# Tencent-RoboticsX/lifelike-agility-and-play

Hardware: NVIDIA H100
Metric: env-steps/sec PMC mocap-tracking (higher is better)
Workload: dtype f32

## Files before the change

lifelike_agility_and_play_b200/csrc/llq_cuda.cu:

```cuda
#include "../../include/llq.h"
#include "../../include/llq_model_layout.h"
#include "llq_kernels.cuh"
#include "llq_step16.cuh"

#include <cmath>
#include <cstdio>
#include <cstdlib>
#include <cstring>
#include <new>
#include <string>
#include <vector>

namespace {

thread_local std::string g_err;
int fail(int code, const std::string& msg) { g_err = msg; return code; }
#define CK(call)                                                                                         \
  do {                                                                                                   \
    cudaError_t e_ = (call);                                                                             \
    if (e_ != cudaSuccess) return fail(LLQ_ECUDA, std::string(#call) + ": " + cudaGetErrorString(e_));   \
  } while (0)

constexpr int kPadFrames = 128;

// ... 48 lines not shown
  P.sim_dt = c.sim_dt; P.frame_dt = h->frame_dt; P.margin = h->margin;
  P.max_steps = c.max_steps; P.cmd_freq_lo = c.cmd_freq_lo; P.cmd_freq_hi = c.cmd_freq_hi; P.push_start_count = c.push_start_count;
  P.push_interval = c.push_interval_steps; P.push_duration = c.push_duration_steps; P.push_enabled = c.push_enabled;
  P.mu_ground = (float)c.ground_friction; P.fr_lo = (float)c.friction_lo; P.fr_hi = (float)c.friction_hi;
  P.ph_lo = (float)c.push_h_lo; P.ph_hi = (float)c.push_h_hi; P.pv_lo = (float)c.push_v_lo; P.pv_hi = (float)c.push_v_hi;
  P.ts_lo = (float)c.target_spd_lo; P.ts_hi = (float)c.target_spd_hi;
  P.knee = c.knee_contacts; P.mu_wheel = (float)(c.ground_friction * c.link_friction); P.aux_r = (float)c.auxiliary_radius;
  P.element_id = c.element_id; P.ww_lo = (float)c.wall_width_lo; P.ww_hi = (float)c.wall_width_hi; P.wg_lo = (float)c.wall_gap_lo;
  P.wg_hi = (float)c.wall_gap_hi; P.hg_lo = (float)c.hole_gap_lo; P.hg_hi = (float)c.hole_gap_hi;
  if (!h->has_obstacles) { P.has_ob = 0; P.ob_hx = P.ob_hy = P.ob_hz = 0.f; }
}

template <typename T> int dalloc(T** p, size_t n) {
  CK(cudaMalloc((void**)p, n * sizeof(T)));
  CK(cudaMemset(*p, 0, n * sizeof(T)));
  return LLQ_OK;
}

int ensure_scratch(llq_handle h, size_t bytes) {
  if (bytes > h->h_scratch_bytes) {
    if (h->h_scratch) cudaFreeHost(h->h_scratch);
    if (h->d_scratch) cudaFree(h->d_scratch);
    h->h_scratch = nullptr; h->d_scratch = nullptr; h->h_scratch_bytes = 0;
    CK(cudaMallocHost(&h->h_scratch, bytes));
    CK(cudaMalloc(&h->d_scratch, bytes));
    h->h_scratch_bytes = h->d_scratch_bytes = bytes;
  }
  return LLQ_OK;
}

llq::MocapDev mocap_dev(llq_handle h) { return llq::MocapDev{h->d_frames, h->d_clip_off, h->n_clips, h->d_ob_table, h->d_ob_off}; }

template <int ENV>
void launch_reset_t(llq_handle h, const llq::EnvArrays& E, const llq::ResetParams& RP, float* obs2, long long ld, cudaStream_t s) {
  constexpr int BLOCK = llq::kResetBlock;
  int threads = 4 * h->cfg.n_envs;
  int grid = (threads + BLOCK - 1) / BLOCK;
  size_t smem = sizeof(double) * (size_t)(h->n_clips > 0 ? h->n_clips : 1);
  llq::pmc_reset_kernel<ENV><<<grid, BLOCK, smem, s>>>(E, mocap_dev(h), h->P, h->d_model, RP, obs2, ld);
}
template <int ENV>
int launch_step16(llq_handle h, const llq::EnvArrays& E, const float* a, float* obs2, long long ld, cudaStream_t s) {
  constexpr int EPB = LLQ16_BLOCK / 16;
  const int grid = (h->cfg.n_envs + EPB - 1) / EPB;
  const size_t smem = sizeof(float) * (EPB * llq::kEnvFloats + (LLQ16_BLOCK / 32) * llq::kATabWarp);
  const unsigned bit = 1u << (16 + ENV);
  if (!(h->smem_attr_set & bit)) {
    CK(cudaFuncSetAttribute(llq::llq_step16_kernel<ENV>, cudaFuncAttributeMaxDynamicSharedMemorySize, (int)smem));
    h->smem_attr_set |= bit;
  }
  llq::llq_step16_kernel<ENV><<<grid, LLQ16_BLOCK, smem, s>>>(E, mocap_dev(h), h->P, h->d_model, h->d_sph, a, obs2, ld, h->d_winner[h->parity],
                                                   (unsigned long long)h->cfg.seed, (long long)h->cfg.global_env_offset, h->record);
  return LLQ_OK;
}
int launch_step(llq_handle h, const llq::EnvArrays& E, const float* a, float* obs2, long long ld, cudaStream_t s) {
  const bool epmc = h->cfg.env_kind == LLQ_ENV_EPMC;
  h->counters[4]++;
  if (epmc && h->cfg.element_id != 0) return launch_step16<3>(h, E, a, obs2, ld, s);
  if (h->cfg.env_kind == LLQ_ENV_SEPMC) return launch_step16<2>(h, E, a, obs2, ld, s);
  return epmc ? launch_step16<1>(h, E, a, obs2, ld, s) : launch_step16<0>(h, E, a, obs2, ld, s);
}
void launch_reset(llq_handle h, const llq::EnvArrays& E, const llq::ResetParams& RP, float* obs2, long long ld, cudaStream_t s) {
  if (h->cfg.env_kind == LLQ_ENV_EPMC && h->cfg.element_id != 0) launch_reset_t<3>(h, E, RP, obs2, ld, s);
  else if (h->cfg.env_kind == LLQ_ENV_EPMC) launch_reset_t<1>(h, E, RP, obs2, ld, s);
  else if (h->cfg.env_kind == LLQ_ENV_SEPMC) launch_reset_t<2>(h, E, RP, obs2, ld, s);
  else launch_reset_t<0>(h, E, RP, obs2, ld, s);
  h->counters[4]++;
}

llq::ResetParams reset_params(llq_handle h, int mode, bool update_table) {
  llq::ResetParams RP{};
  RP.mode = mode; RP.mask = nullptr; RP.clip_in = nullptr; RP.time_in = nullptr;
  RP.seed = h->cfg.seed; RP.gid0 = h->cfg.global_env_offset;
  RP.winner_cur = h->d_winner[h->parity]; RP.winner_next = h->d_winner[h->parity ^ 1];
  RP.avg_old = h->d_avg[h->parity]; RP.avg_new = update_table ? h->d_avg[h->parity ^ 1] : h->d_avg[h->parity];
  RP.prob = h->d_prob; RP.max_steps = h->d_max_steps; RP.factor = h->cfg.prioritized_sample_factor;
  RP.update_table = update_table ? 1 : 0;
  return RP;
}

int check_ready(llq_handle h, bool need_reset) {
  if (!h) return fail(LLQ_EINVAL, "null handle");
  if (!h->has_model) return fail(LLQ_ESTATE, "llq_load_model has not been called");
  if (h->cfg.env_kind == LLQ_ENV_PMC && !h->has_mocap) return fail(LLQ_ESTATE, "llq_load_mocap has not been called");
  if (h->cfg.env_kind != LLQ_ENV_PMC && !h->has_init_state) return fail(LLQ_ESTATE, "llq_set_init_state has not been called");
  if (need_reset && !h->was_reset) return fail(LLQ_ESTATE, "llq_reset has not been called");
  return set_device(h);
}

void copy_item(llq::DampItem& d, const double* s) {
  d.m = (float)s[0];
  for (int i = 0; i < 3; i++) d.c[i] = (float)s[1 + i];
  for (int i = 0; i < 6; i++) d.Ic[i] = (float)s[4 + i];
}

int get_soa_f(llq_handle h, const float* d_src, int width, float* dst) {
  const int n = h->cfg.n_envs;
  int rc = ensure_scratch(h, sizeof(float) * (size_t)width * n);
  if (rc) return rc;
  CK(cudaMemcpyAsync(h->h_scratch, d_src, sizeof(float) * (size_t)width * n, cudaMemcpyDeviceToHost, h->stream));
// ... 287 lines not shown
  const size_t total = (size_t)offsets[n_clips];
  CK(cudaMalloc((void**)&h->d_ob_table, sizeof(double) * 4 * (total ? total : 1)));
  if (total) CK(cudaMemcpy(h->d_ob_table, table, sizeof(double) * 4 * total, cudaMemcpyHostToDevice));
  CK(cudaMalloc((void**)&h->d_ob_off, sizeof(int) * (n_clips + 1)));
  CK(cudaMemcpy(h->d_ob_off, offsets, sizeof(int) * (n_clips + 1), cudaMemcpyHostToDevice));
  h->has_obstacles = true;
  h->P.has_ob = 1; h->P.ob_hx = (float)hx; h->P.ob_hy = (float)hy; h->P.ob_hz = (float)hz;
  return LLQ_OK;
}

static int do_reset(llq_handle h, const uint8_t* mask, const int32_t* clip, const double* time, float* obs) {
  const size_t n = (size_t)h->cfg.n_envs;
  llq::ResetParams RP = reset_params(h, clip ? 2 : 1, false);
  if (mask) {
    std::memcpy(h->h_done, mask, n);
    CK(cudaMemcpyAsync(h->d_mask, h->h_done, n, cudaMemcpyHostToDevice, h->stream));
    RP.mask = h->d_mask;
  }
  if (clip) {
    for (size_t i = 0; i < n; i++) {
      if (mask && !mask[i]) continue;
      if (clip[i] < 0 || clip[i] >= h->n_clips) return fail(LLQ_EINVAL, "clip id out of range");
      int nf = h->clip_off[clip[i] + 1] - h->clip_off[clip[i]];
      if (!(time[i] >= 0) || time[i] >= h->frame_dt * (nf - h->margin - 1)) return fail(LLQ_EINVAL, "reset time outside clip");
    }
    int rc = ensure_scratch(h, n * (sizeof(int) + sizeof(double)));
    if (rc) return rc;
    double* ht = (double*)h->h_scratch; int* hc = (int*)(ht + n);
    std::memcpy(ht, time, n * sizeof(double)); std::memcpy(hc, clip, n * sizeof(int));
    CK(cudaMemcpyAsync(h->d_time_in, ht, n * sizeof(double), cudaMemcpyHostToDevice, h->stream));
    CK(cudaMemcpyAsync(h->d_clip_in, hc, n * sizeof(int), cudaMemcpyHostToDevice, h->stream));
    RP.clip_in = h->d_clip_in; RP.time_in = h->d_time_in;
  }
  launch_reset(h, h->E, RP, nullptr, h->obs_dim, h->stream);
  CK(cudaGetLastError());
  if (obs) CK(cudaMemcpyAsync(h->h_obs, h->E.obs, sizeof(float) * h->obs_dim * n, cudaMemcpyDeviceToHost, h->stream));
  CK(cudaStreamSynchronize(h->stream));
  if (obs) std::memcpy(obs, h->h_obs, sizeof(float) * h->obs_dim * n);
  h->was_reset = true;
  return LLQ_OK;
}

int llq_reset(llq_handle h, const uint8_t* mask, float* obs) {
  int rc = check_ready(h, false);
  if (rc) return rc;
  return do_reset(h, mask, nullptr, nullptr, obs);
}

int llq_reset_to(llq_handle h, const uint8_t* mask, const int32_t* clip, const double* time, float* obs) {
  int rc = check_ready(h, false);
  if (rc) return rc;
  if (h->cfg.env_kind != LLQ_ENV_PMC) return fail(LLQ_EUNSUPPORTED, "llq_reset_to is a PMC (mocap) entry point");
  if (!clip || !time) return fail(LLQ_EINVAL, "null clip/time");
  return do_reset(h, mask, clip, time, obs);
}

int llq_step_ex(llq_handle h, const float* actions, float* obs, int64_t obs_ld, float* reward, uint8_t* done, int io_mode,
                void* stream) {
  int rc = check_ready(h, true);
  if (rc) return rc;
  if (!actions) return fail(LLQ_EINVAL, "null actions");
  const size_t od = (size_t)h->obs_dim;
  if (obs && obs_ld < (int64_t)od) return fail(LLQ_EINVAL, "obs_ld smaller than the observation width");
  if (h->record && io_mode == LLQ_IO_DEVICE && obs && obs_ld < (int64_t)od + 14)
    return fail(LLQ_EINVAL, "record mode needs obs_ld >= observation width + 14 (action 12 | reward | done)");
  const size_t n = (size_t)h->cfg.n_envs;
  llq::EnvArrays E = h->E;
  const float* d_act;
  float* obs2 = nullptr;
  cudaStream_t s = h->stream;
  if (io_mode == LLQ_IO_DEVICE) {
    if (stream) s = (cudaStream_t)stream;
    d_act = actions;
    if (reward) E.reward = reward;
    if (done) E.done = done;
    obs2 = obs;
  } else if (io_mode == LLQ_IO_HOST) {
    std::memcpy(h->h_actions, actions, sizeof(float) * LLQ_ACTION_DIM * n);
    CK(cudaMemcpyAsync(h->d_actions, h->h_actions, sizeof(float) * LLQ_ACTION_DIM * n, cudaMemcpyHostToDevice, s));
    d_act = h->d_actions;
  } else if (io_mode == LLQ_IO_PINNED) {
    CK(cudaMemcpyAsync(h->d_actions, actions, sizeof(float) * LLQ_ACTION_DIM * n, cudaMemcpyHostToDevice, s));
    d_act = h->d_actions;
  } else {
    return fail(LLQ_EINVAL, "bad io_mode");
  }
  if (h->profile) CK(cudaEventRecord(h->ev[0], s));
  rc = launch_step(h, E, d_act, obs2, (long long)obs_ld, s);
  if (rc) return rc;
  if (h->profile) CK(cudaEventRecord(h->ev[1], s));
  llq::ResetParams RP = reset_params(h, h->cfg.auto_reset ? 0 : 3, true);
  launch_reset(h, E, RP, obs2, (long long)obs_ld, s);
  if (h->profile) { CK(cudaEventRecord(h->ev[2], s)); h->ev_valid = true; }
  h->parity ^= 1;
  CK(cudaGetLastError());
  h->counters[0] += (int64_t)n;
  if (io_mode == LLQ_IO_HOST) {
    if (obs) CK(cudaMemcpyAsync(h->h_obs, h->E.obs, sizeof(float) * od * n, cudaMemcpyDeviceToHost, s));
    if (reward) CK(cudaMemcpyAsync(h->h_reward, h->E.reward, sizeof(float) * n, cudaMemcpyDeviceToHost, s));
    if (done) CK(cudaMemcpyAsync(h->h_done, h->E.done, n, cudaMemcpyDeviceToHost, s));
    CK(cudaStreamSynchronize(s));
    if (obs) {
      if ((size_t)obs_ld == od) std::memcpy(obs, h->h_obs, sizeof(float) * od * n);
      else for (size_t i = 0; i < n; i++) std::memcpy(obs + i * obs_ld, h->h_obs + i * od, sizeof(float) * od);
    }
    if (reward) std::memcpy(reward, h->h_reward, sizeof(float) * n);
    if (done) std::memcpy(done, h->h_done, n);
  } else if (io_mode == LLQ_IO_PINNED) {
    if (obs) {
      if ((size_t)obs_ld == od) CK(cudaMemcpyAsync(obs, h->E.obs, sizeof(float) * od * n, cudaMemcpyDeviceToHost, s));
      else CK(cudaMemcpy2DAsync(obs, sizeof(float) * obs_ld, h->E.obs, sizeof(float) * od, sizeof(float) * od, n, cudaMemcpyDeviceToHost, s));
    }
    if (reward) CK(cudaMemcpyAsync(reward, h->E.reward, sizeof(float) * n, cudaMemcpyDeviceToHost, s));
    if (done) CK(cudaMemcpyAsync(done, h->E.done, n, cudaMemcpyDeviceToHost, s));
    CK(cudaStreamSynchronize(s));
  }
  return LLQ_OK;
}

int llq_step(llq_handle h, const float* actions, float* obs, float* reward, uint8_t* done) {
  if (!h) return fail(LLQ_EINVAL, "null handle");
  return llq_step_ex(h, actions, obs, h->obs_dim, reward, done, LLQ_IO_HOST, nullptr);
}

int llq_get_field(llq_handle h, int field, void* dst) {
// ... 151 lines not shown
  if (!h->profile || !h->ev_valid) return fail(LLQ_ESTATE, "profiling is off or no step has run");
  int rc = set_device(h);
  if (rc) return rc;
  CK(cudaEventSynchronize(h->ev[2]));
  float a = 0, b = 0;
  CK(cudaEventElapsedTime(&a, h->ev[0], h->ev[1]));
  CK(cudaEventElapsedTime(&b, h->ev[1], h->ev[2]));
  out[0] = a; out[1] = b;
  return LLQ_OK;
}

int llq_host_alloc(void** out, int64_t bytes) {
  if (!out || bytes <= 0) return fail(LLQ_EINVAL, "bad arguments");
  CK(cudaHostAlloc(out, (size_t)bytes, cudaHostAllocPortable));
  return LLQ_OK;
}
int llq_host_free(void* p) {
  if (p) CK(cudaFreeHost(p));
  return LLQ_OK;
}

int llq_sync(llq_handle h) {
  if (!h) return fail(LLQ_EINVAL, "null handle");
  int rc = set_device(h);
  if (rc) return rc;
  CK(cudaStreamSynchronize(h->stream));
  return LLQ_OK;
}

const char* llq_last_error(void) { return g_err.c_str(); }

}

#ifdef LLQ16_TIMING
extern "C" int llq_debug_timing(void* out, int n_warps) {
  return cudaMemcpyFromSymbol(out, llq::g_t16, (size_t)n_warps * 12 * sizeof(unsigned long long)) == cudaSuccess ? 0 : -1;
}
#endif
```

lifelike_agility_and_play_b200/csrc/llq_kernels.cuh:

```cuda
#pragma once
#include "../../include/llq.h"
#include "llq_math.cuh"
#include <cuda_pipeline.h>
#include <stdint.h>

namespace llq {

constexpr int kObsDim = 207, kObsDimEpmc = 916, kObsDimSepmc = 965, kPropDim = 33, kActDim = 12, kStateDim = 37, kAuxDim = 18;
template <int ENV> struct ObsW { static constexpr int value = (ENV == 1 || ENV == 3) ? kObsDimEpmc : (ENV == 2 ? kObsDimSepmc : kObsDim); };
constexpr int kMaxBoxes = 36, kMaxCand = 12;

constexpr int kNewObs = 120;
constexpr int kSQ = 0, kSQd = 12;
constexpr int kSPropBase = 24;
constexpr int kSAct = kPropDim;
constexpr int kSFuture = 45;
constexpr int kSRot = 45;
constexpr int kSPos = 54;
constexpr int kSTarget = 57;
constexpr int kSTargetSpd = 59;
constexpr int kSPosNorm = 60;
constexpr int kSCorrYaw = 61;
constexpr int kSMaskGrid = 62, kSMaskFront = 64, kSMaskLidar = 66;
constexpr int kSFlag = 57;
// ... 595 lines not shown
        V3 from, d;
        front_ray(sn, j - kOFront, from, d);
        const M3 R = staged_rot(sn);
        const float len = 3.0f * sqrtf(R.a00 * R.a00 + R.a10 * R.a10 + R.a20 * R.a20);
        const float fz = from.z, tz = fz + d.z;
        v = (fz > 0.f && tz < 0.f) ? len * (fz / (fz - tz)) : len;
      } else {
        v = sn[kSTarget + (j - kOTail)];
      }
      obs[(size_t)(env0 + e) * OW + j] = v;
      if (obs2) obs2[(size_t)(env0 + e) * obs2_ld + j] = v;
    }
  }
}

template <int ENV, int EPW = 8>
LLQ_DI void prefetch_history(const float* obs, float* hist_warp, int env0, int n_envs) {
  constexpr int OW = ObsW<ENV>::value;
  const int lane = threadIdx.x & 31;
  for (int idx = lane; idx < EPW * kHist; idx += 32) {
    int e = idx / kHist, t = idx - e * kHist;
    int env = env0 + e < n_envs ? env0 + e : n_envs - 1;
    int j = t < kHistProp ? kPropDim + t : kOPropA + kActDim + (t - kHistProp);
    __pipeline_memcpy_async(hist_warp + idx, obs + (size_t)env * OW + j, 4);
  }
}
LLQ_DI void prefetch_model(const ModelConst* gmodel, ModelConst* smodel, int nthreads) {
  static_assert(sizeof(ModelConst) % 16 == 0, "ModelConst must be a multiple of 16 bytes");
  const float4* src = reinterpret_cast<const float4*>(gmodel);
  float4* dst = reinterpret_cast<float4*>(smodel);
  for (int i = threadIdx.x; i < (int)(sizeof(ModelConst) / 16); i += nthreads) __pipeline_memcpy_async(dst + i, src + i, 16);
}

struct ResetParams {
  int mode; const unsigned char* mask; const int* clip_in; const double* time_in;
  unsigned long long seed; long long gid0;
  int* winner_cur; int* winner_next;
  const double* avg_old; double* avg_new;
  double* prob;
  const double* max_steps;
  double factor;
  int update_table;
};

struct StartPose { Q4 qn, qp; float q[3], qd[3]; V3 lin, ang; };
LLQ_DI StartPose start_pose(const ModelConst& M, int k, double yaw_deg) {
  StartPose s;
  double sn, cs;
  sincos(0.5 * yaw_deg * (3.14159265358979323846 / 180.0), &sn, &cs);
  const float* I0 = M.init_state;
  s.qn = qmul(qnormalize(Q4{I0[3], I0[4], I0[5], I0[6]}), Q4{0.f, 0.f, (float)sn, (float)cs});
#pragma unroll
  for (int i = 0; i < 3; i++) { s.q[i] = I0[13 + 3 * k + i]; s.qd[i] = I0[25 + 3 * k + i]; }
  s.lin = V3{I0[7], I0[8], I0[9]}; s.ang = V3{I0[10], I0[11], I0[12]};
  const Q4 qI = Q4{M.base.qI[0], M.base.qI[1], M.base.qI[2], M.base.qI[3]};
  s.qp = qmul(qnormalize(s.qn), qconj(qI));
  return s;
}

constexpr int kResetBlock = 128;
template <int ENV>
__global__ void __launch_bounds__(kResetBlock) pmc_reset_kernel(EnvArrays E, MocapDev mc, StepParams P, const ModelConst* __restrict__ gmodel,
                                                                ResetParams RP, float* obs2, long long obs2_ld) {
  extern __shared__ double s_cdf[];
  __shared__ __align__(16) ModelConst M;
  __shared__ __align__(16) float s_new[kResetBlock / 4][kNewObs];
  prefetch_model(gmodel, &M, kResetBlock);
  __pipeline_commit();
  const int C = mc.n_clips;
  for (int c = threadIdx.x; c < C; c += kResetBlock) {
    double avg = RP.avg_old[c];
    if (RP.update_table) {
      int w = RP.winner_cur[c];
      if (w >= 0) avg = (double)E.done_reward[w] / RP.max_steps[c];
    }
    s_cdf[c] = avg;
  }
  __syncthreads();
  if (RP.update_table && blockIdx.x == 0)
    for (int c = threadIdx.x; c < C; c += kResetBlock) { RP.avg_new[c] = s_cdf[c]; RP.winner_next[c] = -1; }
  __syncthreads();
  for (int c = threadIdx.x; c < C; c += kResetBlock) s_cdf[c] = pow(1.0 - s_cdf[c], RP.factor);
  __syncthreads();
  __shared__ double s_tot;
  if (threadIdx.x == 0) {
    double tot = 0;
    for (int c = 0; c < C; c++) tot += s_cdf[c];
    s_tot = tot;
  }
  __syncthreads();
  for (int c = threadIdx.x; c < C; c += kResetBlock) {
    const double pc = s_cdf[c] / s_tot;
    s_cdf[c] = pc;
    if (blockIdx.x == 0) RP.prob[c] = pc;
  }
  __syncthreads();
  if (threadIdx.x == 0 && C > 0) {
    double acc = 0;
    for (int c = 0; c < C; c++) { acc += s_cdf[c]; s_cdf[c] = acc; }
    s_tot = s_cdf[C - 1];
  }
  __syncthreads();
  for (int c = threadIdx.x; c < C; c += kResetBlock) s_cdf[c] = s_cdf[c] / s_tot;
  __syncthreads();

  __pipeline_wait_prior(0);
  __syncthreads();
  const int N = P.n_envs;
  const int gtid = blockIdx.x * kResetBlock + threadIdx.x;
  const int env_raw = gtid >> 2;
  const int env = env_raw < N ? env_raw : N - 1;
  const bool valid = env_raw < N;
  const int k = threadIdx.x & 3;
  bool doit = valid;
  if (RP.mode == 3) doit = false;
  else if (RP.mode == 0) doit = doit && E.done[env] != 0;
  else if (RP.mask) doit = doit && (RP.mask[env] != 0 || (ENV == 2 && RP.mask[env ^ 1] != 0));
  const unsigned wm = __ballot_sync(FULL, doit);
  if (wm == 0) return;
  const LegConst& L = M.leg[k];

  if (ENV == 2) {
    const int robot = env & 1;
    const long long ep = E.episode[env & ~1];
    const long long gid = RP.gid0 + (env & ~1);
    double u0[4], u1[4], u2[4];
    stream_uniforms(RP.seed, gid, ep, 1, 0, u0);
    stream_uniforms(RP.seed, gid, ep, 1, 1, u1);
    stream_uniforms(RP.seed, gid, ep, 1, 2, u2);
    const float fix_spd = (float)(0.5 + 2.5 * u0[0]);
    const int wflag = (int)floor(2.0 * u0[1]);
    const double foot_mu = (double)P.fr_lo + u0[2] * ((double)P.fr_hi - (double)P.fr_lo);
    const double px = robot == 0 ? -2.0 + 4.0 * u0[3] : -2.0 + 4.0 * u1[1], py = robot == 0 ? -2.0 + 4.0 * u1[0] : -2.0 + 4.0 * u1[2];
    const double acc0 = E.aux[LLQ_AUX_YAW_ACCUM_DEG * N + (env & ~1)];
    const double yaw_a = fmod(acc0 + 360.0 * u1[3], 360.0), yaw_b = fmod(yaw_a + 360.0 * u2[0], 360.0);
    const StartPose S = start_pose(M, k, robot == 0 ? yaw_a : yaw_b);
    PairState PS = {robot == 0 ? wflag : 1 - wflag, 0, 1, 0, -2.0 + 4.0 * u2[1], -2.0 + 4.0 * u2[2]};
    const bool touch_own = E.aux[LLQ_AUX_FLAG_TOUCH * N + env] != 0.0;
    float* snew = s_new[threadIdx.x >> 2];
    const float* spart = s_new[(threadIdx.x >> 2) ^ 1];
    sepmc_pair_tail(M, L, k, robot, snew, spart, px, py, 0.5, S.qp, S.qn, S.lin, S.ang, S.q, touch_own, fix_spd, RP.seed, gid, ep, PS);
    stage_joints(snew, k, S.q, S.qd);
    int push_draws = 0;
    float pf[3] = {0.f, 0.f, 0.f};
    if (P.push_enabled) push_draws = 1;
    if (doit) {
      write_robot(E, N, env, k, S.q, S.qd, foot_world(L, S.qp, S.q, px, py, 0.5), px, py, 0.5, S.qn, S.lin, S.ang, 0.0);
      write_reset(E, N, env, k, ep + 1);
      if (k == 0) {
        double* A = E.aux;
        A[LLQ_AUX_COUNTER * N + env] = 0; A[LLQ_AUX_WITH_FLAG * N + env] = PS.with_flag; A[LLQ_AUX_FLAG_X * N + env] = PS.flag_x;
        A[LLQ_AUX_FLAG_Y * N + env] = PS.flag_y; A[LLQ_AUX_CONTROL_SPD * N + env] = fix_spd;
// ... 21 lines not shown
    if (ENV == 3) nb0 = generate_corridor(P, RP.seed, gid, ep, E.boxes + (size_t)env * (6 * kMaxBoxes), doit && k == 0, tgx0);
    const StartPose S = start_pose(M, k, yaw_deg);
    const Q4 qn = S.qn;
    float* snew = s_new[threadIdx.x >> 2];
    const M3 Rq = qmat(qnormalize(qn));
    stage_joints(snew, k, S.q, S.qd);
    if (k == 0) {
      stage_pose(snew, Rq, tmul(Rq, S.ang), tmul(Rq, S.lin), V3{0.f, 0.f, 0.5f});
      stage_target(snew, Rq, 0.0, 0.0, 0.5, tgx0, 0.0, target_spd);
    }
    if (ENV == 3) {
      __syncwarp();
      stage_corridor_masks(snew, E.boxes + (size_t)env * (6 * kMaxBoxes), doit ? nb0 : E.nbox[env], k, 0.f, 0.f, 0.5f, atan2f(Rq.a10, Rq.a00));
    }
    if (doit) {
      const Q4 qI = Q4{M.base.qI[0], M.base.qI[1], M.base.qI[2], M.base.qI[3]};
      const V3 f = mul(qmat(qmul(qnormalize(qn), qconj(qI))), foot_in_base(L, S.q[0], S.q[1], S.q[2]));
      write_robot(E, N, env, k, S.q, S.qd, V3{f.x, f.y, 0.5f + f.z}, 0.0, 0.0, 0.5, qn, S.lin, S.ang, 0.0);
      write_reset(E, N, env, k, ep + 1);
      if (k == 0) {
        double* A = E.aux;
        A[LLQ_AUX_COUNTER * N + env] = 0; A[LLQ_AUX_CMD_FREQ * N + env] = cmd_freq; A[LLQ_AUX_TARGET_X * N + env] = tgx0;
        A[LLQ_AUX_TARGET_Y * N + env] = 0.0; A[LLQ_AUX_LAST_POS_DIFF_LEN * N + env] = fabs(tgx0); A[LLQ_AUX_TOTAL_SPD * N + env] = 0.0;
        A[LLQ_AUX_INIT_POS_DIFF_LEN * N + env] = fabs(tgx0);
        if (ENV == 3) E.nbox[env] = nb0;
        A[LLQ_AUX_MAX_SPD * N + env] = 0.0; A[LLQ_AUX_PUSH_COUNT * N + env] = P.push_start_count; A[LLQ_AUX_PUSH_F * N + env] = pf[0];
        A[(LLQ_AUX_PUSH_F + 1) * N + env] = pf[1]; A[(LLQ_AUX_PUSH_F + 2) * N + env] = pf[2];
        A[LLQ_AUX_FOOT_FRICTION * N + env] = foot_mu; A[LLQ_AUX_PUSH_DRAWS * N + env] = push_draws; A[LLQ_AUX_CMD_DRAWS * N + env] = 0;
        A[LLQ_AUX_YAW_ACCUM_DEG * N + env] = yaw_deg;
      }
    }
  } else {
    int clip; double t0;
    long long ep = E.episode[env];
    if (RP.mode == 2) {
      clip = RP.clip_in[env]; t0 = RP.time_in[env];
      if (!doit) { clip = 0; t0 = 0.0; }
    } else {
      long long gid = RP.gid0 + env;
      unsigned c4[4] = {(unsigned)gid, (unsigned)((unsigned long long)gid >> 32), (unsigned)ep, (unsigned)((unsigned long long)ep >> 32)};
      philox4x32_10(c4, (unsigned)RP.seed, (unsigned)(RP.seed >> 32));
      double u1 = ((double)c4[0] + 0.5) * (1.0 / 4294967296.0), u2 = ((double)c4[1] + 0.5) * (1.0 / 4294967296.0);
      clip = C - 1;
      for (int c = 0; c < C; c++) if (s_cdf[c] > u1) { clip = c; break; }
      int nf = mc.clip_off[clip + 1] - mc.clip_off[clip];
      t0 = u2 * (P.frame_dt * (double)(nf - P.margin - 1));
      ep += 1;
    }
    int frame_id = (int)floor(t0 / P.frame_dt);
    double frac = (t0 - frame_id * P.frame_dt) / P.frame_dt;
    {
      const int last = mc.clip_off[clip + 1] - mc.clip_off[clip] - P.margin + 2;
      if (frame_id > last) { frame_id = last; frac = 0.0; }
      if (frame_id < 0) { frame_id = 0; frac = 0.0; }
    }
    const MocapFrame* f0 = mc.frames + mc.clip_off[clip] + frame_id;
    KinBase kb = mocap_base(f0, f0 + 1, frac, P.frame_dt);
    float inv = (float)(1.0 / P.frame_dt), fr = (float)frac;
    float q[3], qd[3];
#pragma unroll
    for (int i = 0; i < 3; i++) {
      float c = f0->q[3 * k + i], n = f0[1].q[3 * k + i];
      q[i] = fmaf(fr, n - c, c);
      qd[i] = (n - c) * inv;
    }
    build_obs_new(mc, P, M, k, clip, frame_id, frac, kb.px, kb.py, kb.pz, kb.q, kb.lin, kb.ang, q, qd, s_new[threadIdx.x >> 2]);
    if (doit) {
      const Q4 qI = Q4{M.base.qI[0], M.base.qI[1], M.base.qI[2], M.base.qI[3]};
      const V3 fd = foot_world(L, qmul(qnormalize(kb.q), qconj(qI)), q, kb.px, kb.py, kb.pz);
      write_robot(E, N, env, k, q, qd, fd, kb.px, kb.py, kb.pz, kb.q, kb.lin, kb.ang, t0);
      write_reset(E, N, env, k, ep);
#pragma unroll
      for (int i = 0; i < 3; i++) { E.kin[(13 + 3 * k + i) * N + env] = q[i]; E.kin[(25 + 3 * k + i) * N + env] = qd[i]; }
      if (k == 0) {
        const float b[10] = {kb.q.x, kb.q.y, kb.q.z, kb.q.w, kb.lin.x, kb.lin.y, kb.lin.z, kb.ang.x, kb.ang.y, kb.ang.z};
        E.kin[env] = (float)kb.px; E.kin[N + env] = (float)kb.py; E.kin[2 * N + env] = (float)kb.pz;
#pragma unroll
        for (int i = 0; i < 10; i++) E.kin[(3 + i) * N + env] = b[i];
        E.clip[env] = clip;
        E.ob_id[env] = 0;
      }
    }
  }
  __syncwarp();
  unsigned rows = 0;
#pragma unroll
  for (int e = 0; e < 8; e++) if ((wm >> (4 * e)) & 1u) rows |= 1u << e;
  const int warp_env0 = (blockIdx.x * kResetBlock + (threadIdx.x & ~31)) >> 2;
  emit_obs_rows<ENV>(E.obs, obs2, obs2_ld, s_new[(threadIdx.x & ~31) >> 2], s_new[0], warp_env0, N, 1, rows, E.boxes);
}

}
```

lifelike_agility_and_play_b200/csrc/llq_step16.cuh:

```cuda
#pragma once
#include "llq_kernels.cuh"

namespace llq {

#ifndef LLQ16_BLOCK
#define LLQ16_BLOCK 256
#endif
#ifndef LLQ16_MINB
#define LLQ16_MINB 4
#endif
constexpr int kMaxSph = 32, kMaxCon = 8, kMaxLim = 8;
struct SphConst { float c[3]; float r; float mu_link; int leg; int depth; int foot; };
struct alignas(16) SphTable { int n; int rule; int pad[2]; SphConst s[kMaxSph]; };

constexpr int kLinkTab = 12 * 8;
constexpr int kLegTab = 4 * 48;
constexpr int kConW = 20, kConTab = kMaxCon * kConW;
constexpr int kLimTab = kMaxLim * 4;
constexpr int kRowW = 12, kRowTab = 32 * kRowW;
constexpr int kEnvTab = 56;
constexpr int kATabWarp = 32 * 32;
constexpr int kEnvFloats = 944;
static_assert(kLinkTab + kLegTab + kConTab + kLimTab + kRowTab + kEnvTab <= kEnvFloats && kEnvFloats % 32 == 16, "per-env table layout");

// ... 530 lines not shown
        Aw[LLQ_AUX_TARGET_ANGLE * N + env] = target_angle; Aw[LLQ_AUX_LAST_POS_DIFF_LEN * N + env] = last_len;
        Aw[LLQ_AUX_TOTAL_SPD * N + env] = total_spd; Aw[LLQ_AUX_MAX_SPD * N + env] = max_spd;
        Aw[LLQ_AUX_PUSH_COUNT * N + env] = push_count; Aw[LLQ_AUX_PUSH_F * N + env] = pf[0]; Aw[(LLQ_AUX_PUSH_F + 1) * N + env] = pf[1]; Aw[(LLQ_AUX_PUSH_F + 2) * N + env] = pf[2];
        Aw[LLQ_AUX_PUSH_DRAWS * N + env] = push_draws; Aw[LLQ_AUX_CMD_DRAWS * N + env] = cmd_draws;
      }
    }
  }
  if (record && obs2 && wr) {
    float* row = obs2 + (size_t)env * obs2_ld + ObsW<ENV>::value - (record == 2 ? (long long)N * obs2_ld : 0ll);
#pragma unroll
    for (int t = 0; t < 3; t++) row[3 * k + t] = act_src[3 * k + t];
    if (k == 0) { row[12] = rew_out; row[13] = done ? 1.f : 0.f; }
  }
  {
    const unsigned dm = __ballot_sync(FULL, valid && k == 0 && done);
    if ((threadIdx.x & 31) == 0 && dm) atomicAdd(&E.counters[1], (unsigned long long)__popc(dm));
  }
}

template <int ENV>
__global__ void __launch_bounds__(LLQ16_BLOCK, LLQ16_MINB * 128 / LLQ16_BLOCK) llq_step16_kernel(EnvArrays E, MocapDev mc, StepParams P, const ModelConst* __restrict__ gmodel,
                                                            const SphTable* __restrict__ gsph, const float* __restrict__ actions,
                                                            float* obs2, long long obs2_ld, int* __restrict__ winner,
                                                            unsigned long long seed, long long gid0, int record) {
  constexpr int BLOCK = LLQ16_BLOCK, EPB = BLOCK / 16;
  constexpr int EPT = (EPB + 7) / 8 * 8;
  static_assert(BLOCK % 32 == 0 && EPB <= 32, "whole warps; one lane per env in the pairing");
  __shared__ __align__(16) ModelConst M;
  __shared__ __align__(16) SphTable ST;
  __shared__ __align__(16) float s_new[EPT][kNewObs];
  __shared__ __align__(16) float s_hist[EPT][kHist];
  __shared__ __align__(16) int s_cnt[32];
  extern __shared__ __align__(16) float s_env_dyn[];
  const int tid = threadIdx.x;
  const int N = P.n_envs;
  prefetch_model(gmodel, &M, BLOCK);
  {
    const float4* src = reinterpret_cast<const float4*>(gsph);
    float4* dst = reinterpret_cast<float4*>(&ST);
    for (int t = tid; t < (int)(sizeof(SphTable) / 16); t += BLOCK) __pipeline_memcpy_async(dst + t, src + t, 16);
  }
  __pipeline_commit();
  const int warp_env0 = blockIdx.x * EPB + ((tid >> 5) << 1);
  prefetch_history<ENV, 2>(E.obs, s_hist[(tid >> 5) << 1], warp_env0, N);
  __pipeline_commit();
  __pipeline_wait_prior(1);
  __syncthreads();

  const int l16 = tid & 15, k = l16 & 3, i = l16 >> 2, el = tid >> 4;
  const int env_raw = blockIdx.x * EPB + el;
  const int env = env_raw < N ? env_raw : N - 1;
  const bool valid = env_raw < N;
  const LegConst& L = M.leg[k];
  const V3 r0 = ld3(L.j[0].r), r1 = ld3(L.j[1].r), r2 = ld3(L.j[2].r);
  float* const linktab = s_env_dyn + el * kEnvFloats;
  float* const legtab = linktab + kLinkTab;
  float* const contab = legtab + kLegTab;
  float* const limtab = contab + kConTab;
  float* const rowtab = limtab + kLimTab;
  float* const scr = rowtab;
  float* const envtab = rowtab + kRowTab;
  float* const s_atab = s_env_dyn + EPB * kEnvFloats;
  for (int col = 0; col < 32; col++) s_atab[(tid >> 5) * kATabWarp + col * 32 + (tid & 31)] = 0.f;
  for (int t = l16; t < kConTab; t += 16) contab[t] = 0.f;
  unsigned lowmask = 0;
#pragma unroll
// ... 35 lines not shown
    const double* A = E.aux;
    push_count = (int)A[LLQ_AUX_PUSH_COUNT * N + env];
    pf[0] = (float)A[LLQ_AUX_PUSH_F * N + env]; pf[1] = (float)A[(LLQ_AUX_PUSH_F + 1) * N + env]; pf[2] = (float)A[(LLQ_AUX_PUSH_F + 2) * N + env];
    mu_env = P.mu_ground * (float)A[LLQ_AUX_FOOT_FRICTION * N + env]; push_draws = (int)A[LLQ_AUX_PUSH_DRAWS * N + env];
    epi = E.episode[ENV == 2 ? env & ~1 : env] - 1;
    if (ENV == 2) { PS.flag_x = A[LLQ_AUX_FLAG_X * N + env]; PS.flag_y = A[LLQ_AUX_FLAG_Y * N + env]; }
  }
  int n_cand = 0;
  float* s_cand = nullptr;
  if (ENV == 3) {
    s_cand = s_new[el];
    const float* bxs = E.boxes + (size_t)env * (6 * kMaxBoxes);
    unsigned long long m = box_mask(bxs, E.nbox[env], k, (float)px, (float)py, (float)pz, 0.8f, false);
    int c = 0;
    while (m && c < kMaxCand) {
      const int j = __ffsll((long long)m) - 1;
      m &= m - 1;
      if ((c & 3) == k && i == 0) {
#pragma unroll
        for (int t = 0; t < 6; t++) s_cand[6 * c + t] = bxs[6 * j + t];
      }
      c++;
    }
    n_cand = c;
    __syncwarp();
  }
  const Q4 qI = Q4{M.base.qI[0], M.base.qI[1], M.base.qI[2], M.base.qI[3]};
  Q4 qp = qmul(qnormalize(qb), qconj(qI));
  unsigned n_contact_rows = 0, n_limit_rows = 0, n_overflow = 0;
  bool bad = false;
  const float mu_foot = ENV != 0 ? mu_env : P.mu;

  T16_DECL;
  for (int sub = 0; sub < P.substeps; sub++) {
    T16_MARK(5);
    const float dt = P.dt;
    bool push_on = false;
    if (ENV == 2 && P.push_enabled) {
      push_count += 1;
      if (push_count > 0) {
        if (push_count % P.push_interval == 0) { push_draws += 1; push_count = 0; }
        if (push_count < P.push_duration) {
          int d = push_draws - 1 + robot;
          epmc_randomize_push(P, seed, pair_gid, epi, d, pf);
          push_draws += 2;
          push_on = true;
        }
      }
    }
    if ((ENV == 1 || ENV == 3) && P.push_enabled) {
      push_count += 1;
      if (push_count > 0) {
        if (push_count % P.push_interval == 0) { epmc_randomize_push(P, seed, gid0 + env, epi, push_draws, pf); push_count = 0; }
        push_on = push_count < P.push_duration;
      }
    }
    V3 wbs, vbs;
    {
    const M3 R = qmat(qp);
    float c1, s1, c2, s2, c3, s3;
    {
      float so, co;
      llq_sincosf(i == 0 ? q[0] : (i == 1 ? -q[1] : -q[2]), &so, &co);
      c1 = __shfl_sync(FULL, co, k, 16); s1 = __shfl_sync(FULL, so, k, 16);
      c2 = __shfl_sync(FULL, co, k + 4, 16); s2 = __shfl_sync(FULL, so, k + 4, 16);
      c3 = __shfl_sync(FULL, co, k + 8, 16); s3 = __shfl_sync(FULL, so, k + 8, 16);
// ... 479 lines not shown
    }
    __syncwarp();
    T16_MARK(3);
    {
      V3 dw = mul(R, V3{dvb[0], dvb[1], dvb[2]}), dv = mul(R, V3{dvb[3], dvb[4], dvb[5]});
      ww = V3{clampf(ww.x + dw.x, -P.vmax, P.vmax), clampf(ww.y + dw.y, -P.vmax, P.vmax), clampf(ww.z + dw.z, -P.vmax, P.vmax)};
      vw = V3{clampf(vw.x + dv.x, -P.vmax, P.vmax), clampf(vw.y + dv.y, -P.vmax, P.vmax), clampf(vw.z + dv.z, -P.vmax, P.vmax)};
#pragma unroll
      for (int t = 0; t < 3; t++) {
        qd[t] = clampf(qd[t] + dvl[t], -P.vmax, P.vmax);
        q[t] = fmaf(qd[t], dt, q[t]);
      }
      px += (double)vw.x * P.sim_dt; py += (double)vw.y * P.sim_dt; pz += (double)vw.z * P.sim_dt;
      float fa = norm3(ww);
      float sc;
      sc = 0.5f * dt - dt * dt * dt * 0.020833333333f * fa * fa;
      float sh, chh;
      llq_sincosf(0.5f * fa * dt, &sh, &chh);
      if (!(fa < 0.001f)) sc = sh / fa;
      Q4 dq = Q4{sc * ww.x, sc * ww.y, sc * ww.z, chh};
      qp = qnormalize(qmul(dq, qp));
    }
    bad = bad || !(fabsf(qd[0]) <= P.vmax) || !(fabsf(ww.x) <= P.vmax) || !(fabsf(vw.x) <= P.vmax) || !isfinite(q[0] + q[1] + q[2]);
    if (ENV == 0 && sub == P.substeps - 1) {
      frame_id = (int)floor(time / P.frame_dt);
      frame_frac = (time - frame_id * P.frame_dt) / P.frame_dt;
      const int last = mc.clip_off[clip + 1] - mc.clip_off[clip] - P.margin + 2;
      if (frame_id > last) { frame_id = last; frame_frac = 0.0; }
      if (frame_id < 0) { frame_id = 0; frame_frac = 0.0; }
    }
    time += P.sim_dt;
  }
  __syncwarp();

  {
    int bi = bad ? 1 : 0;
    bi |= __shfl_xor_sync(FULL, bi, 1); bi |= __shfl_xor_sync(FULL, bi, 2); bi |= __shfl_xor_sync(FULL, bi, 4); bi |= __shfl_xor_sync(FULL, bi, 8);
    bad = bi != 0;
  }
  if (valid) {
    if (l16 < nsph) E.warm[(size_t)l16 * N + env] = warm[0];
    if (16 + l16 < nsph) E.warm[(size_t)(16 + l16) * N + env] = warm[1];
  }
  {
    TailState* T = reinterpret_cast<TailState*>(rowtab);
    if (l16 == 0) {
      T->px = px; T->py = py; T->pz = pz; T->time = time; T->frame_frac = frame_frac;
      T->frame_id = frame_id; T->ob_id = ob_id; T->push_count = push_count; T->push_draws = push_draws;
      T->pf[0] = pf[0]; T->pf[1] = pf[1]; T->pf[2] = pf[2];
      T->qp[0] = qp.x; T->qp[1] = qp.y; T->qp[2] = qp.z; T->qp[3] = qp.w;
      T->vw[0] = vw.x; T->vw[1] = vw.y; T->vw[2] = vw.z; T->ww[0] = ww.x; T->ww[1] = ww.y; T->ww[2] = ww.z;
    }
    int fl = (bad ? 1 : 0) | (ob_hit ? 2 : 0) | (touch_own ? 4 : 0) | (tag ? 8 : 0);
    fl |= __shfl_xor_sync(FULL, fl, 1); fl |= __shfl_xor_sync(FULL, fl, 2);
    if (l16 == 0) T->flags = fl;
    if (i == 0) {
#pragma unroll
      for (int t = 0; t < 3; t++) { T->q[3 * k + t] = q[t]; T->qd[3 * k + t] = qd[t]; }
    }
  }
  {
    unsigned cr = n_contact_rows, lr = n_limit_rows, ov = n_overflow;
    if (!valid) { cr = 0; lr = 0; ov = 0; }
#pragma unroll
    for (int o = 16; o > 0; o >>= 1) { cr += __shfl_xor_sync(FULL, cr, o); lr += __shfl_xor_sync(FULL, lr, o); ov += __shfl_xor_sync(FULL, ov, o); }
    if ((threadIdx.x & 31) == 0) {
      if (cr) atomicAdd(&E.counters[2], (unsigned long long)cr);
      if (lr) atomicAdd(&E.counters[3], (unsigned long long)lr);
      if (ov) atomicAdd(&E.counters[5], (unsigned long long)ov);
    }
  }
  __pipeline_wait_prior(0);
  __syncthreads();
  if (tid < 4 * EPT) {
    const int tel = tid >> 2, tk = tid & 3;
    const bool tval = tel < EPB && blockIdx.x * EPB + tel < N;
    const int tsrc = tel < EPB ? tel : EPB - 1;
    const int tenv_raw = blockIdx.x * EPB + tsrc;
    const float* tbase = s_env_dyn + tsrc * kEnvFloats;
    step_tail<ENV>(E, mc, P, M, s_new[0], s_hist[0], *reinterpret_cast<const TailState*>(tbase + (rowtab - linktab)),
                        tbase + (envtab - linktab) + 44, obs2, obs2_ld, winner, seed, gid0, record, tel, tk, tenv_raw < N ? tenv_raw : N - 1, tval);
  }
  __syncthreads();
  emit_obs_rows<ENV, 2>(E.obs, obs2, obs2_ld, s_new[(tid >> 5) << 1], s_hist[(tid >> 5) << 1], warp_env0, N, 0, 0x3u, E.boxes);
#ifdef LLQ16_TIMING
  T16_MARK(4);
  t16_[7] = clock64() - t16_s;
  if ((tid & 31) == 0) {
    const int gw = blockIdx.x * (BLOCK / 32) + (tid >> 5);
    if (gw < 16384) for (int t = 0; t < 12; t++) g_t16[gw * 12 + t] = (unsigned long long)t16_[t];
  }
#endif
}

}
```

Measured before the change: 16.80 million.

## Overlap reset kernel prologue with step kernel via programmatic dependent launch

Launches the reset kernel with programmatic stream serialization after the step kernel, and has the step kernel trigger dependents once its substep loop ends. The reset kernel does its model prefetch, RNG draws and clip-offset staging before waiting on the step grid. The clip-probability setup is merged into fewer passes, and when the CDF is sorted a binary search replaces the linear clip search. It also prefetches mocap frames into L1 and adds optional phase-clock instrumentation. Correctness depends on every read of step outputs happening after griddepcontrol.wait.

Result: faster. 17.12 million (median of 6 runs) (+1.9%).

```diff
diff --git a/lifelike_agility_and_play_b200/csrc/llq_cuda.cu b/lifelike_agility_and_play_b200/csrc/llq_cuda.cu
--- a/lifelike_agility_and_play_b200/csrc/llq_cuda.cu
+++ b/lifelike_agility_and_play_b200/csrc/llq_cuda.cu
@@ -104,12 +104,18 @@
 llq::MocapDev mocap_dev(llq_handle h) { return llq::MocapDev{h->d_frames, h->d_clip_off, h->n_clips, h->d_ob_table, h->d_ob_off}; }
 
 template <int ENV>
-void launch_reset_t(llq_handle h, const llq::EnvArrays& E, const llq::ResetParams& RP, float* obs2, long long ld, cudaStream_t s) {
+cudaError_t launch_reset_t(llq_handle h, const llq::EnvArrays& E, const llq::ResetParams& RP, float* obs2, long long ld, cudaStream_t s,
+                           bool after_step) {
   constexpr int BLOCK = llq::kResetBlock;
   int threads = 4 * h->cfg.n_envs;
-  int grid = (threads + BLOCK - 1) / BLOCK;
-  size_t smem = sizeof(double) * (size_t)(h->n_clips > 0 ? h->n_clips : 1);
-  llq::pmc_reset_kernel<ENV><<<grid, BLOCK, smem, s>>>(E, mocap_dev(h), h->P, h->d_model, RP, obs2, ld);
+  cudaLaunchAttribute attr;
+  attr.id = cudaLaunchAttributeProgrammaticStreamSerialization;
+  attr.val.programmaticStreamSerializationAllowed = 1;
+  cudaLaunchConfig_t lc = {};
+  lc.gridDim = dim3((threads + BLOCK - 1) / BLOCK); lc.blockDim = dim3(BLOCK);
+  lc.dynamicSmemBytes = (sizeof(double) + sizeof(int)) * (size_t)h->n_clips + sizeof(int) + sizeof(double); lc.stream = s;
+  lc.attrs = &attr; lc.numAttrs = after_step ? 1 : 0;
+  return cudaLaunchKernelEx(&lc, llq::pmc_reset_kernel<ENV>, E, mocap_dev(h), h->P, (const llq::ModelConst*)h->d_model, RP, obs2, ld);
 }
 template <int ENV>
 int launch_step16(llq_handle h, const llq::EnvArrays& E, const float* a, float* obs2, long long ld, cudaStream_t s) {
@@ -132,12 +138,14 @@
   if (h->cfg.env_kind == LLQ_ENV_SEPMC) return launch_step16<2>(h, E, a, obs2, ld, s);
   return epmc ? launch_step16<1>(h, E, a, obs2, ld, s) : launch_step16<0>(h, E, a, obs2, ld, s);
 }
-void launch_reset(llq_handle h, const llq::EnvArrays& E, const llq::ResetParams& RP, float* obs2, long long ld, cudaStream_t s) {
-  if (h->cfg.env_kind == LLQ_ENV_EPMC && h->cfg.element_id != 0) launch_reset_t<3>(h, E, RP, obs2, ld, s);
-  else if (h->cfg.env_kind == LLQ_ENV_EPMC) launch_reset_t<1>(h, E, RP, obs2, ld, s);
-  else if (h->cfg.env_kind == LLQ_ENV_SEPMC) launch_reset_t<2>(h, E, RP, obs2, ld, s);
-  else launch_reset_t<0>(h, E, RP, obs2, ld, s);
+int launch_reset(llq_handle h, const llq::EnvArrays& E, const llq::ResetParams& RP, float* obs2, long long ld, cudaStream_t s,
+                 bool after_step) {
   h->counters[4]++;
+  if (h->cfg.env_kind == LLQ_ENV_EPMC && h->cfg.element_id != 0) CK(launch_reset_t<3>(h, E, RP, obs2, ld, s, after_step));
+  else if (h->cfg.env_kind == LLQ_ENV_EPMC) CK(launch_reset_t<1>(h, E, RP, obs2, ld, s, after_step));
+  else if (h->cfg.env_kind == LLQ_ENV_SEPMC) CK(launch_reset_t<2>(h, E, RP, obs2, ld, s, after_step));
+  else CK(launch_reset_t<0>(h, E, RP, obs2, ld, s, after_step));
+  return LLQ_OK;
 }
 
 llq::ResetParams reset_params(llq_handle h, int mode, bool update_table) {
@@ -491,8 +499,8 @@
     CK(cudaMemcpyAsync(h->d_clip_in, hc, n * sizeof(int), cudaMemcpyHostToDevice, h->stream));
     RP.clip_in = h->d_clip_in; RP.time_in = h->d_time_in;
   }
-  launch_reset(h, h->E, RP, nullptr, h->obs_dim, h->stream);
-  CK(cudaGetLastError());
+  int rc = launch_reset(h, h->E, RP, nullptr, h->obs_dim, h->stream, false);
+  if (rc) return rc;
   if (obs) CK(cudaMemcpyAsync(h->h_obs, h->E.obs, sizeof(float) * h->obs_dim * n, cudaMemcpyDeviceToHost, h->stream));
   CK(cudaStreamSynchronize(h->stream));
   if (obs) std::memcpy(obs, h->h_obs, sizeof(float) * h->obs_dim * n);
@@ -549,7 +557,8 @@
   if (rc) return rc;
   if (h->profile) CK(cudaEventRecord(h->ev[1], s));
   llq::ResetParams RP = reset_params(h, h->cfg.auto_reset ? 0 : 3, true);
-  launch_reset(h, E, RP, obs2, (long long)obs_ld, s);
+  rc = launch_reset(h, E, RP, obs2, (long long)obs_ld, s, !h->profile);
+  if (rc) return rc;
   if (h->profile) { CK(cudaEventRecord(h->ev[2], s)); h->ev_valid = true; }
   h->parity ^= 1;
   CK(cudaGetLastError());
@@ -767,6 +776,15 @@
 
 }
 
+#ifdef LLQ_PHASE_CLOCKS
+extern "C" int llq_debug_phases(void* out) {
+  constexpr size_t n = 2 * llq::kPhaseCtas * llq::kPhaseSlots;
+  static unsigned long long zero[n];
+  if (cudaMemcpyFromSymbol(out, llq::g_phase, n * sizeof(unsigned long long)) != cudaSuccess) return -1;
+  return cudaMemcpyToSymbol(llq::g_phase, zero, n * sizeof(unsigned long long)) == cudaSuccess ? 0 : -1;
+}
+#endif
+
 #ifdef LLQ16_TIMING
 extern "C" int llq_debug_timing(void* out, int n_warps) {
   return cudaMemcpyFromSymbol(out, llq::g_t16, (size_t)n_warps * 12 * sizeof(unsigned long long)) == cudaSuccess ? 0 : -1;
diff --git a/lifelike_agility_and_play_b200/csrc/llq_kernels.cuh b/lifelike_agility_and_play_b200/csrc/llq_kernels.cuh
--- a/lifelike_agility_and_play_b200/csrc/llq_kernels.cuh
+++ b/lifelike_agility_and_play_b200/csrc/llq_kernels.cuh
@@ -651,6 +651,22 @@
   for (int i = threadIdx.x; i < (int)(sizeof(ModelConst) / 16); i += nthreads) __pipeline_memcpy_async(dst + i, src + i, 16);
 }
 
+LLQ_DI void allow_dependent_launch() { asm volatile("griddepcontrol.launch_dependents;" ::: "memory"); }
+LLQ_DI void wait_for_prerequisite_grid() { asm volatile("griddepcontrol.wait;" ::: "memory"); }
+
+#ifdef LLQ_PHASE_CLOCKS
+constexpr int kPhaseCtas = 1024, kPhaseSlots = 8;
+__device__ unsigned long long g_phase[2][kPhaseCtas][kPhaseSlots];
+LLQ_DI void phase_mark(int kernel, int slot) {
+  unsigned long long t;
+  asm volatile("mov.u64 %0, %%globaltimer;" : "=l"(t));
+  if ((threadIdx.x & 31) == 0 && blockIdx.x < kPhaseCtas) atomicMax(&g_phase[kernel][blockIdx.x][slot], t);
+}
+#define PHASE_MARK(kernel, slot) phase_mark(kernel, slot)
+#else
+#define PHASE_MARK(kernel, slot)
+#endif
+
 struct ResetParams {
   int mode; const unsigned char* mask; const int* clip_in; const double* time_in;
   unsigned long long seed; long long gid0;
@@ -677,6 +693,43 @@
   return s;
 }
 
+LLQ_DI double sequential_sum(const double* v, int n) {
+  double s = 0.0;
+  for (int c0 = 0; c0 < n; c0 += 8) {
+    double x[8];
+#pragma unroll
+    for (int j = 0; j < 8; j++) x[j] = c0 + j < n ? v[c0 + j] : 0.0;
+#pragma unroll
+    for (int j = 0; j < 8; j++) if (c0 + j < n) s += x[j];
+  }
+  return s;
+}
+LLQ_DI bool sequential_cumsum(double* v, int n) {
+  double acc = 0.0, prev = -INFINITY;
+  bool sorted = true;
+  for (int c0 = 0; c0 < n; c0 += 8) {
+    double x[8];
+#pragma unroll
+    for (int j = 0; j < 8; j++) x[j] = c0 + j < n ? v[c0 + j] : 0.0;
+#pragma unroll
+    for (int j = 0; j < 8; j++)
+      if (c0 + j < n) {
+        acc += x[j];
+        v[c0 + j] = acc;
+        sorted &= acc >= prev;
+        prev = acc;
+      }
+  }
+  return sorted && acc > 0.0 && acc < INFINITY;
+}
+
+LLQ_DI void prefetch_frame_pair(const MocapFrame* f) {
+  const char* b = reinterpret_cast<const char*>(f);
+  asm volatile("prefetch.global.L1 [%0];" ::"l"(b));
+  asm volatile("prefetch.global.L1 [%0];" ::"l"(b + 128));
+  asm volatile("prefetch.global.L1 [%0];" ::"l"(b + 2 * sizeof(MocapFrame) - 1));
+}
+
 constexpr int kResetBlock = 128;
 template <int ENV>
 __global__ void __launch_bounds__(kResetBlock) pmc_reset_kernel(EnvArrays E, MocapDev mc, StepParams P, const ModelConst* __restrict__ gmodel,
@@ -684,59 +737,76 @@
   extern __shared__ double s_cdf[];
   __shared__ __align__(16) ModelConst M;
   __shared__ __align__(16) float s_new[kResetBlock / 4][kNewObs];
+  PHASE_MARK(1, 0);
   prefetch_model(gmodel, &M, kResetBlock);
   __pipeline_commit();
   const int C = mc.n_clips;
-  for (int c = threadIdx.x; c < C; c += kResetBlock) {
-    double avg = RP.avg_old[c];
-    if (RP.update_table) {
-      int w = RP.winner_cur[c];
-      if (w >= 0) avg = (double)E.done_reward[w] / RP.max_steps[c];
-    }
-    s_cdf[c] = avg;
-  }
-  __syncthreads();
-  if (RP.update_table && blockIdx.x == 0)
-    for (int c = threadIdx.x; c < C; c += kResetBlock) { RP.avg_new[c] = s_cdf[c]; RP.winner_next[c] = -1; }
-  __syncthreads();
-  for (int c = threadIdx.x; c < C; c += kResetBlock) s_cdf[c] = pow(1.0 - s_cdf[c], RP.factor);
-  __syncthreads();
-  __shared__ double s_tot;
-  if (threadIdx.x == 0) {
-    double tot = 0;
-    for (int c = 0; c < C; c++) tot += s_cdf[c];
-    s_tot = tot;
-  }
-  __syncthreads();
-  for (int c = threadIdx.x; c < C; c += kResetBlock) {
-    const double pc = s_cdf[c] / s_tot;
-    s_cdf[c] = pc;
-    if (blockIdx.x == 0) RP.prob[c] = pc;
-  }
-  __syncthreads();
-  if (threadIdx.x == 0 && C > 0) {
-    double acc = 0;
-    for (int c = 0; c < C; c++) { acc += s_cdf[c]; s_cdf[c] = acc; }
-    s_tot = s_cdf[C - 1];
-  }
-  __syncthreads();
-  for (int c = threadIdx.x; c < C; c += kResetBlock) s_cdf[c] = s_cdf[c] / s_tot;
-  __syncthreads();
-
-  __pipeline_wait_prior(0);
-  __syncthreads();
   const int N = P.n_envs;
   const int gtid = blockIdx.x * kResetBlock + threadIdx.x;
   const int env_raw = gtid >> 2;
   const int env = env_raw < N ? env_raw : N - 1;
   const bool valid = env_raw < N;
   const int k = threadIdx.x & 3;
+  long long ep_pmc = 0;
+  double u1 = 0.0, u2 = 0.0;
+  if (ENV == 0) {
+    ep_pmc = E.episode[env];
+    if (RP.mode != 2) {
+      const long long gid = RP.gid0 + env;
+      unsigned c4[4] = {(unsigned)gid, (unsigned)((unsigned long long)gid >> 32), (unsigned)ep_pmc, (unsigned)((unsigned long long)ep_pmc >> 32)};
+      philox4x32_10(c4, (unsigned)RP.seed, (unsigned)(RP.seed >> 32));
+      u1 = ((double)c4[0] + 0.5) * (1.0 / 4294967296.0); u2 = ((double)c4[1] + 0.5) * (1.0 / 4294967296.0);
+    }
+  }
+  const int c_first = threadIdx.x;
+  double avg_first = 0.0, ms_first = 1.0;
+  if (c_first < C) { avg_first = RP.avg_old[c_first]; ms_first = RP.max_steps[c_first]; }
+  int* const s_off = reinterpret_cast<int*>(s_cdf + C);
+  MocapDev mcs = mc;
+  if (ENV == 0) {
+    for (int i = threadIdx.x; i <= C; i += kResetBlock) __pipeline_memcpy_async(s_off + i, mc.clip_off + i, 4);
+    mcs.clip_off = s_off;
+  }
+  __pipeline_commit();
+  wait_for_prerequisite_grid();
   bool doit = valid;
   if (RP.mode == 3) doit = false;
   else if (RP.mode == 0) doit = doit && E.done[env] != 0;
   else if (RP.mask) doit = doit && (RP.mask[env] != 0 || (ENV == 2 && RP.mask[env ^ 1] != 0));
+  __shared__ double s_tot;
+  __shared__ int s_sorted;
+  for (int c = threadIdx.x; c < C; c += kResetBlock) {
+    double avg = c == c_first ? avg_first : RP.avg_old[c];
+    if (RP.update_table) {
+      const int w = RP.winner_cur[c];
+      if (w >= 0) avg = (double)E.done_reward[w] / (c == c_first ? ms_first : RP.max_steps[c]);
+      if (blockIdx.x == 0) { RP.avg_new[c] = avg; RP.winner_next[c] = -1; }
+    }
+    s_cdf[c] = pow(1.0 - avg, RP.factor);
+  }
+  __syncthreads();
+  if (threadIdx.x == 0) s_tot = sequential_sum(s_cdf, C);
+  __syncthreads();
+  for (int c = threadIdx.x; c < C; c += kResetBlock) {
+    const double pc = s_cdf[c] / s_tot;
+    s_cdf[c] = pc;
+    if (blockIdx.x == 0) RP.prob[c] = pc;
+  }
+  __syncthreads();
+  if (threadIdx.x == 0 && C > 0) {
+    s_sorted = sequential_cumsum(s_cdf, C);
+    s_tot = s_cdf[C - 1];
+  }
+  __syncthreads();
+  for (int c = threadIdx.x; c < C; c += kResetBlock) s_cdf[c] = s_cdf[c] / s_tot;
+  __pipeline_wait_prior(0);
+  __syncthreads();
+  PHASE_MARK(1, 1);
   const unsigned wm = __ballot_sync(FULL, doit);
-  if (wm == 0) return;
+  if (wm == 0) {
+    PHASE_MARK(1, 2); PHASE_MARK(1, 3);
+    return;
+  }
   const LegConst& L = M.leg[k];
 
   if (ENV == 2) {
@@ -824,29 +894,39 @@
     }
   } else {
     int clip; double t0;
-    long long ep = E.episode[env];
+    long long ep = ep_pmc;
     if (RP.mode == 2) {
       clip = RP.clip_in[env]; t0 = RP.time_in[env];
       if (!doit) { clip = 0; t0 = 0.0; }
     } else {
-      long long gid = RP.gid0 + env;
-      unsigned c4[4] = {(unsigned)gid, (unsigned)((unsigned long long)gid >> 32), (unsigned)ep, (unsigned)((unsigned long long)ep >> 32)};
-      philox4x32_10(c4, (unsigned)RP.seed, (unsigned)(RP.seed >> 32));
-      double u1 = ((double)c4[0] + 0.5) * (1.0 / 4294967296.0), u2 = ((double)c4[1] + 0.5) * (1.0 / 4294967296.0);
       clip = C - 1;
-      for (int c = 0; c < C; c++) if (s_cdf[c] > u1) { clip = c; break; }
-      int nf = mc.clip_off[clip + 1] - mc.clip_off[clip];
+      if (s_sorted) {
+        int lo = 0, hi = C;
+        while (lo < hi) {
+          const int mid = (lo + hi) >> 1;
+          if (s_cdf[mid] > u1) hi = mid; else lo = mid + 1;
+        }
+        if (lo < C) clip = lo;
+      } else {
+        for (int c = 0; c < C; c++) if (s_cdf[c] > u1) { clip = c; break; }
+      }
+      int nf = mcs.clip_off[clip + 1] - mcs.clip_off[clip];
       t0 = u2 * (P.frame_dt * (double)(nf - P.margin - 1));
       ep += 1;
     }
     int frame_id = (int)floor(t0 / P.frame_dt);
     double frac = (t0 - frame_id * P.frame_dt) / P.frame_dt;
     {
-      const int last = mc.clip_off[clip + 1] - mc.clip_off[clip] - P.margin + 2;
+      const int last = mcs.clip_off[clip + 1] - mcs.clip_off[clip] - P.margin + 2;
       if (frame_id > last) { frame_id = last; frac = 0.0; }
       if (frame_id < 0) { frame_id = 0; frac = 0.0; }
     }
-    const MocapFrame* f0 = mc.frames + mc.clip_off[clip] + frame_id;
+    const MocapFrame* f0 = mcs.frames + mcs.clip_off[clip] + frame_id;
+    {
+      const double tf = k == 0 ? 1. / 30. : (k == 1 ? 1. / 15. : (k == 2 ? 1. / 3. : 1.));
+      prefetch_frame_pair(f0);
+      prefetch_frame_pair(f0 + (int)(frac + tf / P.frame_dt));
+    }
     KinBase kb = mocap_base(f0, f0 + 1, frac, P.frame_dt);
     float inv = (float)(1.0 / P.frame_dt), fr = (float)frac;
     float q[3], qd[3];
@@ -856,7 +936,7 @@
       q[i] = fmaf(fr, n - c, c);
       qd[i] = (n - c) * inv;
     }
-    build_obs_new(mc, P, M, k, clip, frame_id, frac, kb.px, kb.py, kb.pz, kb.q, kb.lin, kb.ang, q, qd, s_new[threadIdx.x >> 2]);
+    build_obs_new(mcs, P, M, k, clip, frame_id, frac, kb.px, kb.py, kb.pz, kb.q, kb.lin, kb.ang, q, qd, s_new[threadIdx.x >> 2]);
     if (doit) {
       const Q4 qI = Q4{M.base.qI[0], M.base.qI[1], M.base.qI[2], M.base.qI[3]};
       const V3 fd = foot_world(L, qmul(qnormalize(kb.q), qconj(qI)), q, kb.px, kb.py, kb.pz);
@@ -875,11 +955,13 @@
     }
   }
   __syncwarp();
+  PHASE_MARK(1, 2);
   unsigned rows = 0;
 #pragma unroll
   for (int e = 0; e < 8; e++) if ((wm >> (4 * e)) & 1u) rows |= 1u << e;
   const int warp_env0 = (blockIdx.x * kResetBlock + (threadIdx.x & ~31)) >> 2;
   emit_obs_rows<ENV>(E.obs, obs2, obs2_ld, s_new[(threadIdx.x & ~31) >> 2], s_new[0], warp_env0, N, 1, rows, E.boxes);
-}
-
-}
+  PHASE_MARK(1, 3);
+}
+
+}
diff --git a/lifelike_agility_and_play_b200/csrc/llq_step16.cuh b/lifelike_agility_and_play_b200/csrc/llq_step16.cuh
--- a/lifelike_agility_and_play_b200/csrc/llq_step16.cuh
+++ b/lifelike_agility_and_play_b200/csrc/llq_step16.cuh
@@ -586,6 +586,7 @@
   __shared__ __align__(16) float s_hist[EPT][kHist];
   __shared__ __align__(16) int s_cnt[32];
   extern __shared__ __align__(16) float s_env_dyn[];
+  PHASE_MARK(0, 0);
   const int tid = threadIdx.x;
   const int N = P.n_envs;
   prefetch_model(gmodel, &M, BLOCK);
@@ -687,6 +688,7 @@
   const float mu_foot = ENV != 0 ? mu_env : P.mu;
 
   T16_DECL;
+  PHASE_MARK(0, 1);
   for (int sub = 0; sub < P.substeps; sub++) {
     T16_MARK(5);
     const float dt = P.dt;
@@ -1232,6 +1234,8 @@
     time += P.sim_dt;
   }
   __syncwarp();
+  PHASE_MARK(0, 2);
+  allow_dependent_launch();
 
   {
     int bi = bad ? 1 : 0;
@@ -1282,7 +1286,9 @@
                         tbase + (envtab - linktab) + 44, obs2, obs2_ld, winner, seed, gid0, record, tel, tk, tenv_raw < N ? tenv_raw : N - 1, tval);
   }
   __syncthreads();
+  PHASE_MARK(0, 3);
   emit_obs_rows<ENV, 2>(E.obs, obs2, obs2_ld, s_new[(tid >> 5) << 1], s_hist[(tid >> 5) << 1], warp_env0, N, 0, 0x3u, E.boxes);
+  PHASE_MARK(0, 4);
 #ifdef LLQ16_TIMING
   T16_MARK(4);
   t16_[7] = clock64() - t16_s;
```
